# MPEGGroup/mpeg-pcc-tmc2

Hardware: AMD Instinct MI355X
Metric: encoder patch+image-gen frames/sec, longdress_vox10 32-frame GOF (higher is better)
Workload: dtype int32/f64

## Files before the change

mpeg-pcc-tmc2_amd/csrc/kdtree_device.hip:

```cpp
#include <algorithm>
#include <cstring>

#include "internal.h"

namespace tmc2 {
namespace {

constexpr uint32_t kNone      = 0xFFFFFFFFu;
constexpr int      kBlock     = 256;
constexpr int      kWaves     = kBlock / 64;
constexpr int      kScanTile  = kBlock * 8;
constexpr int      kLeafMax   = 10;
constexpr int      kMaxLevels = 64;

struct BuildSeg {
  uint32_t begin, end;
  uint32_t node, parent;
  int32_t  mn[3], mx[3];
  int16_t  lo[3], hi[3];
  uint8_t  side, pdim;
  uint8_t  split, cutDim;
  int32_t  cut;
  uint32_t mid;
  uint32_t slot;
// ... 199 lines not shown
#pragma unroll
          for ( int j = 0; j < 4; ++j ) {
            const uint32_t i = base + j * blockDim.x + threadIdx.x;
            if ( i < count ) {
              const int o = i < idx ? 0 : 6;
              if ( o == 0 ) {
                r[0] = min( r[0], int32_t( p[j].x ) ), r[1] = min( r[1], int32_t( p[j].y ) ), r[2] = min( r[2], int32_t( p[j].z ) );
                r[3] = max( r[3], int32_t( p[j].x ) ), r[4] = max( r[4], int32_t( p[j].y ) ), r[5] = max( r[5], int32_t( p[j].z ) );
              } else {
                r[6] = min( r[6], int32_t( p[j].x ) ), r[7] = min( r[7], int32_t( p[j].y ) ), r[8] = min( r[8], int32_t( p[j].z ) );
                r[9] = max( r[9], int32_t( p[j].x ) ), r[10] = max( r[10], int32_t( p[j].y ) ), r[11] = max( r[11], int32_t( p[j].z ) );
              }
            }
          }
        }
#pragma unroll
        for ( int off = 32; off > 0; off >>= 1 )
#pragma unroll
          for ( int k = 0; k < 12; ++k ) {
            const int32_t o = __shfl_xor( r[k], off, 64 );
            r[k]            = ( k % 6 ) < 3 ? min( r[k], o ) : max( r[k], o );
          }
        if ( lane == 0 )
          for ( int k = 0; k < 12; ++k ) red[wave][k] = r[k];
        __syncthreads();
        if ( threadIdx.x == 0 ) {
          for ( int w = 0; w < kHugeWaves; ++w )
            for ( int k = 0; k < 12; ++k ) r[k] = ( k % 6 ) < 3 ? min( r[k], red[w][k] ) : max( r[k], red[w][k] );
          const uint32_t id0 = atomicAdd( a.nodeCount, 2u );
          KdNode         nd;
          nd.a = int32_t( id0 ), nd.b = int32_t( id0 + 1 ), nd.divlow = int16_t( r[3 + rule.dim] ), nd.divhigh = int16_t( r[6 + rule.dim] ),
          nd.dim = rule.dim;
          a.nodes[q.node] = nd;
          HugeNode child[2];
          child[0].begin = q.begin, child[0].end = q.begin + idx, child[0].node = id0;
          child[1].begin = q.begin + idx, child[1].end = q.end, child[1].node = id0 + 1;
          for ( int c = 0; c < 2; ++c ) {
            child[c].depth = uint16_t( q.depth + 1 );
            for ( int d = 0; d < 3; ++d )
              child[c].lo[d] = lo[d], child[c].hi[d] = hi[d], child[c].mn[d] = int16_t( r[6 * c + d] ), child[c].mx[d] = int16_t( r[6 * c + 3 + d] );
          }
          const int16_t cut = int16_t( rule.cut );
          if ( rule.dim == 0 ) child[0].hi[0] = cut, child[1].lo[0] = cut;
          if ( rule.dim == 1 ) child[0].hi[1] = cut, child[1].lo[1] = cut;
          if ( rule.dim == 2 ) child[0].hi[2] = cut, child[1].lo[2] = cut;
          for ( int c = 0; c < 2; ++c ) {
            const uint32_t cc = child[c].end - child[c].begin, level = seg.level + child[c].depth;
            if ( cc <= uint32_t( kLeafMax ) ) {
              KdNode leaf;
              leaf.a = int32_t( seg.begin + child[c].begin ), leaf.b = int32_t( seg.begin + child[c].end ), leaf.divlow = leaf.divhigh = 0,
              leaf.dim = -1;
              a.nodes[child[c].node] = leaf;
              atomicMax( a.finishDepth, level + 1u );
            } else if ( cc <= a.retireMax ) {
              RetiredSeg rs;
              rs.begin = seg.begin + child[c].begin, rs.end = seg.begin + child[c].end, rs.node = child[c].node, rs.level = level, rs.root = 0;
              for ( int d = 0; d < 3; ++d ) rs.lo[d] = child[c].lo[d], rs.hi[d] = child[c].hi[d];
              a.retired[atomicAdd( a.retiredCount, 1u )] = rs;
            } else {
              sNode[cur ^ 1][sCount[cur ^ 1]++] = child[c];
            }
          }
        }
        __syncthreads();
      }
      if ( threadIdx.x == 0 ) sCount[cur] = 0;
      cur ^= 1;
      __syncthreads();
    }
  }
}

constexpr int      kPieceMax  = 4096;
constexpr int      kPieceRecs = kPieceMax / ( kLeafMax + 1 ) + 2;
constexpr uint16_t kNoRec     = 0xFFFFu;
constexpr uint32_t kNoKey     = 0xFFFFFFFFu;

struct alignas( 8 ) PieceRec {
  uint16_t begin, end;
  int16_t  cut;
  uint8_t  dim, unused0;
  uint16_t edge1, rb1;
  uint16_t edge2, rb2;
  uint16_t mid;
  uint16_t child[2];
  uint16_t unused1;
  uint32_t node;
  int32_t  lmax, rmin;
  int16_t  lo[3], hi[3];
  int32_t  mn[3], mx[3];
};
static_assert( sizeof( PieceRec ) == 72, "PieceRec layout" );
struct PieceHot0 {
  uint32_t be, dc;
};
struct PieceHot1 {
  uint32_t e1rb1, e2rb2;
};
struct PieceHot2 {
  uint32_t midc0, c1;
};

__device__ __forceinline__ void pieceBarrier() { asm volatile( "s_waitcnt lgkmcnt(0)\n\ts_barrier" ::: "memory" ); }

typedef short pkShort2 __attribute__( ( ext_vector_type( 2 ) ) );
__device__ __forceinline__ uint32_t pkMin( uint32_t a, uint32_t b ) {
  return __builtin_bit_cast( uint32_t, __builtin_elementwise_min( __builtin_bit_cast( pkShort2, a ), __builtin_bit_cast( pkShort2, b ) ) );
}
__device__ __forceinline__ uint32_t pkMax( uint32_t a, uint32_t b ) {
  return __builtin_bit_cast( uint32_t, __builtin_elementwise_max( __builtin_bit_cast( pkShort2, a ), __builtin_bit_cast( pkShort2, b ) ) );
}
__device__ __forceinline__ uint32_t pk2( int lo16, int hi16 ) { return ( uint32_t( lo16 ) & 0xFFFFu ) | ( uint32_t( hi16 ) << 16 ); }
__device__ __forceinline__ int      pkLo( uint32_t v ) { return int( int16_t( v & 0xFFFFu ) ); }
__device__ __forceinline__ int      pkHi( uint32_t v ) { return int( int16_t( v >> 16 ) ); }

template <int WAVES>
__device__ __forceinline__ uint32_t pieceScan( uint32_t v, uint32_t* waveTot ) {
  const int lane = threadIdx.x & 63, wave = threadIdx.x >> 6;
  uint32_t  inc  = v;
#pragma unroll
  for ( int off = 1; off < 64; off <<= 1 ) {
    const uint32_t t = __shfl_up( inc, off, 64 );
    if ( lane >= off ) inc += t;
  }
  if ( lane == 63 ) waveTot[wave] = inc;
  pieceBarrier();
  uint32_t before = 0;
#pragma unroll
  for ( int w = 0; w < WAVES; w += 4 ) {
    const uint4 t = *reinterpret_cast<const uint4*>( waveTot + w );
    before += ( w + 0 < wave ? t.x : 0u ) + ( w + 1 < wave ? t.y : 0u ) + ( w + 2 < wave ? t.z : 0u ) + ( w + 3 < wave ? t.w : 0u );
  }
  return before + inc - v;
}

__device__ __forceinline__ bool waveSegMinMaxPacked( uint32_t key, uint32_t& A, uint32_t& B, uint32_t& C, int lane ) {
#pragma unroll
  for ( int off = 1; off < 64; off <<= 1 ) {
    const uint32_t ok = __shfl_down( key, off, 64 );
    const uint32_t oa = __shfl_down( A, off, 64 ), ob = __shfl_down( B, off, 64 ), oc = __shfl_down( C, off, 64 );
    if ( lane + off < 64 && ok == key ) A = pkMin( A, oa ), B = pkMax( B, ob ), C = pkMin( C, oc );
  }
  const uint32_t pk = __shfl_up( key, 1, 64 );
  return key != kNoKey && ( lane == 0 || pk != key );
}

__device__ __forceinline__ void ldsMin( int32_t* slot, int32_t v ) {
  if ( v < *reinterpret_cast<volatile int32_t*>( slot ) ) atomicMin( slot, v );
}
__device__ __forceinline__ void ldsMax( int32_t* slot, int32_t v ) {
  if ( v > *reinterpret_cast<volatile int32_t*>( slot ) ) atomicMax( slot, v );
}


struct LvSeg {
  uint32_t begin, end;
  uint32_t cutInfo;
  uint32_t edge1;
  uint32_t slot;
  uint32_t childNode;
  uint32_t node, parent;
  int16_t  lo[3], hi[3];
  uint8_t  side, pdim;
  uint16_t unused;
  int32_t  mn[3], mx[3];
};

constexpr int kLandBlock = 256;
constexpr int kLandRounds = 2;
struct LvPartial {
  uint32_t slot;
  uint32_t v[6];
  uint32_t unused;
};

__device__ __forceinline__ void lvReport( LvSeg* child, int mnx, int mny, int mnz, int mxx, int mxy, int mxz ) {
  if ( mnx < loadStaleOk( &child->mn[0] ) ) atomicMin( &child->mn[0], mnx );
  if ( mny < loadStaleOk( &child->mn[1] ) ) atomicMin( &child->mn[1], mny );
  if ( mnz < loadStaleOk( &child->mn[2] ) ) atomicMin( &child->mn[2], mnz );
  if ( mxx > loadStaleOk( &child->mx[0] ) ) atomicMax( &child->mx[0], mxx );
  if ( mxy > loadStaleOk( &child->mx[1] ) ) atomicMax( &child->mx[1], mxy );
  if ( mxz > loadStaleOk( &child->mx[2] ) ) atomicMax( &child->mx[2], mxz );
}

__device__ __forceinline__ uint32_t lvPrefix( const uint32_t* __restrict__ loc, const uint32_t* sums, uint32_t tiles, uint32_t i, uint32_t n ) {
  return i < n ? loc[i] + sums[i / kScanTile] : sums[tiles];
}

__device__ __forceinline__ uint32_t lvPartner( const uint16_t* __restrict__ list, const uint32_t* sums, uint32_t from, uint32_t to, uint32_t G ) {
  uint32_t lo = from / kScanTile, hi = ( to - 1u ) / kScanTile;
  while ( lo < hi ) {
    const uint32_t mid = ( lo + hi + 1u ) / 2u;
    if ( mid * kScanTile - sums[mid] <= G )
      lo = mid;
    else
      hi = mid - 1u;
  }
  return lo * kScanTile + list[size_t( lo ) * kScanTile + ( G - ( lo * kScanTile - sums[lo] ) )];
}

__global__ __launch_bounds__( kBlock ) void lvInitKernel( BuildArgs a ) {
  __shared__ int blockRange[6 * kWaves];
  const uint32_t n = a.n, gsize = gridDim.x * blockDim.x;
  const int      lane = threadIdx.x & 63, wave = threadIdx.x >> 6;
  int mnx = 0x7FFFFFFF, mny = mnx, mnz = mnx, mxx = int( 0x80000000 ), mxy = mxx, mxz = mxx;
  for ( uint32_t i = blockIdx.x * blockDim.x + threadIdx.x; i < n; i += gsize ) {
    const Pt p = a.pts[i];
    a.P[i]     = p;
    a.perm[i]  = i;
    a.seg[i]   = 0;
    mnx = min( mnx, int( p.x ) ), mny = min( mny, int( p.y ) ), mnz = min( mnz, int( p.z ) );
    mxx = max( mxx, int( p.x ) ), mxy = max( mxy, int( p.y ) ), mxz = max( mxz, int( p.z ) );
  }
#pragma unroll
  for ( int off = 32; off > 0; off >>= 1 ) {
    mnx = min( mnx, __shfl_xor( mnx, off, 64 ) ), mny = min( mny, __shfl_xor( mny, off, 64 ) ), mnz = min( mnz, __shfl_xor( mnz, off, 64 ) );
    mxx = max( mxx, __shfl_xor( mxx, off, 64 ) ), mxy = max( mxy, __shfl_xor( mxy, off, 64 ) ), mxz = max( mxz, __shfl_xor( mxz, off, 64 ) );
  }
  if ( lane == 0 ) {
    int* w = blockRange + 6 * wave;
    w[0] = mnx, w[1] = mny, w[2] = mnz, w[3] = mxx, w[4] = mxy, w[5] = mxz;
  }
  __syncthreads();
  if ( threadIdx.x < 6 ) {
    int v = blockRange[threadIdx.x];
    for ( int w = 1; w < kWaves; ++w ) v = threadIdx.x < 3 ? min( v, blockRange[6 * w + threadIdx.x] ) : max( v, blockRange[6 * w + threadIdx.x] );
    int32_t* slot = threadIdx.x < 3 ? &a.lvA[0].mn[threadIdx.x] : &a.lvA[0].mx[threadIdx.x - 3];
    if ( threadIdx.x < 3 ) {
      if ( v < loadStaleOk( slot ) ) atomicMin( slot, v );
    } else {
      if ( v > loadStaleOk( slot ) ) atomicMax( slot, v );
    }
  }
}
__global__ void lvRootKernel( BuildArgs a ) {
  if ( threadIdx.x < kMaxLevels + 16 ) a.counts[threadIdx.x] = 0;
  __syncthreads();
  if ( threadIdx.x != 0 ) return;
  LvSeg r{};
  r.begin = 0, r.end = a.n, r.node = 0, r.parent = kNone;
  for ( int d = 0; d < 3; ++d ) r.mn[d] = 0x7FFFFFFF, r.mx[d] = int32_t( 0x80000000 );
  a.lvA[0]     = r;
  a.counts[0]  = 1;
  *a.nodeCount = 1;
}

constexpr int kDecideThreads = 1024;
constexpr int kDecideRng     = 2000;
__global__ __launch_bounds__( kDecideThreads ) void lvDecideKernel( BuildArgs a, uint32_t level ) {
  __shared__ uint32_t waveTot[kDecideThreads / 64];
  __shared__ uint32_t sCarry;
  __shared__ int32_t  sRng[kDecideRng][6];
  LvSeg*         cur   = ( level & 1 ) ? a.lvB : a.lvA;
  const uint32_t count = a.counts[level], nodeBase = *a.nodeCount;
  const int      lane = threadIdx.x & 63, wave = threadIdx.x >> 6;
  if ( threadIdx.x == 0 ) sCarry = 0;
  const bool inLds = level > 0 && count <= a.decideRng;
  if ( inLds ) {
    for ( uint32_t t = threadIdx.x; t < count * 6u; t += kDecideThreads ) sRng[t / 6u][t % 6u] = ( t % 6u ) < 3u ? 0x7FFFFFFF : int32_t( 0x80000000 );
    __syncthreads();
  }
  if ( level > 0 ) {
    const uint32_t nPart = ( a.n + uint32_t( kLandBlock * kLandRounds ) - 1u ) / uint32_t( kLandBlock * kLandRounds );
    for ( uint32_t base = 0; base < nPart; base += kDecideThreads ) {
      const uint32_t t = base + threadIdx.x;
      LvPartial      pt;
      pt.slot = kNone;
      if ( t < nPart ) pt = a.partial[t];
#pragma unroll
      for ( int c = 0; c < 2; ++c ) {
        uint32_t A = pt.v[3 * c], B = pt.v[3 * c + 1], C = pt.v[3 * c + 2];
        if ( waveSegMinMaxPacked( pt.slot == kNone ? kNoKey : pt.slot, A, B, C, lane ) ) {
          if ( inLds ) {
            int32_t* r = sRng[pt.slot + c];
            ldsMin( &r[0], pkLo( A ) ), ldsMin( &r[1], pkHi( A ) ), ldsMin( &r[2], pkLo( C ) );
            ldsMax( &r[3], pkLo( B ) ), ldsMax( &r[4], pkHi( B ) ), ldsMax( &r[5], ~pkHi( C ) );
          } else {
            lvReport( cur + pt.slot + c, pkLo( A ), pkHi( A ), pkLo( C ), pkLo( B ), pkHi( B ), ~pkHi( C ) );
          }
        }
      }
    }
    if ( !inLds ) asm volatile( "s_waitcnt vmcnt(0)" ::: "memory" );
  }
  __syncthreads();
  for ( uint32_t base = 0; base < count; base += kDecideThreads ) {
    const uint32_t s     = base + threadIdx.x;
    uint32_t       split = 0;
    LvSeg*         q     = cur + s;
    if ( s < count ) {
      const bool root = q->parent == kNone;
      int32_t    mn[3], mx[3], lo[3], hi[3];
#pragma unroll
      for ( int d = 0; d < 3; ++d ) {
        mn[d] = __hip_atomic_load( &q->mn[d], __ATOMIC_RELAXED, __HIP_MEMORY_SCOPE_AGENT );
        mx[d] = __hip_atomic_load( &q->mx[d], __ATOMIC_RELAXED, __HIP_MEMORY_SCOPE_AGENT );
        if ( inLds ) mn[d] = min( mn[d], sRng[s][d] ), mx[d] = max( mx[d], sRng[s][3 + d] );
        lo[d] = root ? mn[d] : int32_t( q->lo[d] );
        hi[d] = root ? mx[d] : int32_t( q->hi[d] );
      }
      if ( root ) {
        for ( int d = 0; d < 3; ++d ) a.rootBox[d] = mn[d], a.rootBox[3 + d] = mx[d];
      } else {
        const int pd = q->pdim;
        if ( q->side == 0 )
          a.nodes[q->parent].divlow = int16_t( pd == 0 ? mx[0] : ( pd == 1 ? mx[1] : mx[2] ) );
// ... 173 lines not shown
    if ( i == b ) q->edge1 = edge;
    if ( i >= edge || coordOf( pi, int( ( ci >> 16 ) & 0xFFu ) ) < int32_t( int16_t( ci & 0xFFFFu ) ) ) continue;
    const uint32_t r  = li + lvSums[i / kScanTile] - rb;
    const uint32_t j  = lvPartner( a.list, lvSums, edge, e, ( e - re ) - 1u - r );
    const Pt       pj = a.P[j];
    a.P[i]            = pj;
    a.P[j]            = pi;
    const uint32_t u  = a.perm[i];
    a.perm[i]         = a.perm[j];
    a.perm[j]         = u;
  }
}

__global__ __launch_bounds__( kLandBlock ) void lvSwapTwoKernel( BuildArgs a, uint32_t level ) {
  extern __shared__ uint32_t lvSums[];
  const uint32_t n = a.n, tiles = a.tiles;
  const int      lane  = threadIdx.x & 63;
  LvSeg*         cur  = ( level & 1 ) ? a.lvB : a.lvA;
  LvSeg*         next = ( level & 1 ) ? a.lvA : a.lvB;
  lvLoadSums<kLandBlock>( lvSums, a.tile2, tiles );
  const uint32_t nRound = ( n + uint32_t( kLandBlock ) - 1u ) & ~( uint32_t( kLandBlock ) - 1u );
  __shared__ uint32_t blockSeg;
  __shared__ uint32_t red[kLandBlock / 64][6];
  __shared__ uint32_t accV[6], accSlot;
  const int wave = threadIdx.x >> 6;
  constexpr uint32_t kChunk = uint32_t( kLandBlock ) * kLandRounds;
  for ( uint32_t c0 = blockIdx.x * kChunk; c0 < nRound; c0 += gridDim.x * kChunk ) {
  if ( threadIdx.x == 0 ) accSlot = kNone;
  for ( uint32_t i0 = c0; i0 < min( c0 + kChunk, nRound ); i0 += kLandBlock ) {
    const uint32_t i   = i0 + threadIdx.x;
    uint32_t       key = kNoKey;
    uint32_t       A = pk2( 0x7FFF, 0x7FFF ), B = pk2( -0x8000, -0x8000 ), C = pk2( 0x7FFF, 0x7FFF );
    uint32_t       A2 = A, B2 = B, C2 = C;
    bool           moved = false;
    uint32_t       s = kNone, slot = 0;
    if ( i < n ) {
      s           = a.seg[i];
      uint32_t to = kNone;
      if ( s != kNone ) {
        LvSeg*         q  = cur + s;
        const uint32_t ci = q->cutInfo;
        if ( ci >> 24 ) {
          const uint32_t b = q->begin, e = q->end, e1 = q->edge1;
          slot               = q->slot;
          const int      dim = int( ( ci >> 16 ) & 0xFFu );
          const int32_t  cut = int32_t( int16_t( ci & 0xFFFFu ) );
          Pt             pi  = a.P[i];
          const uint32_t li  = a.loc2[i];
          const uint32_t rb = lvPrefix( a.loc2, lvSums, tiles, e1, n ), re = lvPrefix( a.loc2, lvSums, tiles, e, n );
          const uint32_t e2   = e1 + ( ( e - e1 ) - ( re - rb ) );
          const uint32_t cnt  = e - b, half = cnt / 2, lim1 = e1 - b, lim2 = e2 - b;
          const uint32_t idx  = lim1 > half ? lim1 : ( lim2 < half ? lim2 : half );
          const uint32_t mid  = b + idx;
          if ( i == b ) {
            KdNode nd;
            nd.a = int32_t( q->childNode ), nd.b = int32_t( q->childNode + 1u ), nd.divlow = nd.divhigh = 0, nd.dim = dim;
            a.nodes[q->node] = nd;
            for ( int c = 0; c < 2; ++c ) {
              LvSeg* ch = next + slot + c;
              ch->begin = c ? mid : b, ch->end = c ? e : mid, ch->cutInfo = 0, ch->edge1 = 0, ch->slot = 0, ch->childNode = 0;
              ch->node = q->childNode + c, ch->parent = q->node, ch->side = uint8_t( c ), ch->pdim = uint8_t( dim ), ch->unused = 0;
              for ( int d = 0; d < 3; ++d ) ch->lo[d] = q->lo[d], ch->hi[d] = q->hi[d];
              if ( c == 0 ) {
                if ( dim == 0 ) ch->hi[0] = int16_t( cut );
                if ( dim == 1 ) ch->hi[1] = int16_t( cut );
                if ( dim == 2 ) ch->hi[2] = int16_t( cut );
              } else {
                if ( dim == 0 ) ch->lo[0] = int16_t( cut );
                if ( dim == 1 ) ch->lo[1] = int16_t( cut );
                if ( dim == 2 ) ch->lo[2] = int16_t( cut );
              }
            }
          }
          const int32_t x = coordOf( pi, dim );
          to              = slot + ( i >= mid ? 1u : 0u );
          key             = to;
          if ( i >= e1 && i < e2 && x > cut ) {
            const uint32_t r  = li + lvSums[i / kScanTile] - rb;
            const uint32_t j  = lvPartner( a.list, lvSums, e2, e, ( e - re ) - 1u - r );
            const Pt       pj = a.P[j];
            a.P[i]            = pj;
            a.P[j]            = pi;
            const uint32_t u  = a.perm[i];
            a.perm[i]         = a.perm[j];
            a.perm[j]         = u;
            moved             = true;
            A2 = pk2( pi.x, pi.y ), B2 = A2, C2 = pk2( pi.z, ~int( pi.z ) );
            pi = pj;
          }
          if ( !( i >= e2 && x <= cut ) ) A = pk2( pi.x, pi.y ), B = A, C = pk2( pi.z, ~int( pi.z ) );
        }
        a.seg[i] = to;
      }
    }
    if ( threadIdx.x == 0 ) blockSeg = s;
    __syncthreads();
    const bool uniform = __syncthreads_and( s == blockSeg ) != 0;
    if ( uniform ) {
      const bool anything = __syncthreads_or( key != kNoKey ) != 0;
      if ( anything ) {
        uint32_t v[6];
        const bool right = key != kNoKey && key != slot;
        v[0] = right || key == kNoKey ? pk2( 0x7FFF, 0x7FFF ) : A, v[1] = right || key == kNoKey ? pk2( -0x8000, -0x8000 ) : B,
        v[2] = right || key == kNoKey ? pk2( 0x7FFF, 0x7FFF ) : C;
        v[3] = pkMin( right ? A : pk2( 0x7FFF, 0x7FFF ), A2 ), v[4] = pkMax( right ? B : pk2( -0x8000, -0x8000 ), B2 ),
        v[5] = pkMin( right ? C : pk2( 0x7FFF, 0x7FFF ), C2 );
#pragma unroll
        for ( int off = 32; off > 0; off >>= 1 ) {
          v[0] = pkMin( v[0], __shfl_xor( v[0], off, 64 ) ), v[1] = pkMax( v[1], __shfl_xor( v[1], off, 64 ) ), v[2] = pkMin( v[2], __shfl_xor( v[2], off, 64 ) );
          v[3] = pkMin( v[3], __shfl_xor( v[3], off, 64 ) ), v[4] = pkMax( v[4], __shfl_xor( v[4], off, 64 ) ), v[5] = pkMin( v[5], __shfl_xor( v[5], off, 64 ) );
        }
        if ( lane == 0 )
          for ( int k = 0; k < 6; ++k ) red[wave][k] = v[k];
        __syncthreads();
        if ( threadIdx.x == 0 ) {
          uint32_t x[6];
          for ( int k = 0; k < 6; ++k ) {
            x[k] = red[0][k];
            for ( int w = 1; w < kLandBlock / 64; ++w ) x[k] = ( k % 3 ) == 1 ? pkMax( x[k], red[w][k] ) : pkMin( x[k], red[w][k] );
          }
          if ( accSlot != kNone && accSlot != slot ) {
            for ( int c = 0; c < 2; ++c )
              lvReport( next + accSlot + c, pkLo( accV[3 * c] ), pkHi( accV[3 * c] ), pkLo( accV[3 * c + 2] ), pkLo( accV[3 * c + 1] ), pkHi( accV[3 * c + 1] ),
                        ~pkHi( accV[3 * c + 2] ) );
            accSlot = kNone;
          }
          for ( int k = 0; k < 6; ++k ) accV[k] = accSlot == kNone ? x[k] : ( ( k % 3 ) == 1 ? pkMax( accV[k], x[k] ) : pkMin( accV[k], x[k] ) );
          accSlot = slot;
        }
      }
      __syncthreads();
      continue;
    }
    if ( moved ) lvReport( next + slot + 1u, pkLo( A2 ), pkHi( A2 ), pkLo( C2 ), pkLo( A2 ), pkHi( A2 ), pkLo( C2 ) );
    if ( waveSegMinMaxPacked( key, A, B, C, lane ) )
      lvReport( next + key, pkLo( A ), pkHi( A ), pkLo( C ), pkLo( B ), pkHi( B ), ~pkHi( C ) );
  }
  __syncthreads();
  if ( threadIdx.x == 0 ) {
    LvPartial pt;
    pt.slot = accSlot, pt.unused = 0;
    for ( int k = 0; k < 6; ++k ) pt.v[k] = accV[k];
    a.partial[c0 / kChunk] = pt;
  }
  __syncthreads();
  }
}

constexpr size_t kPieceLdsBytes = size_t( kPieceMax ) * ( sizeof( Pt ) + 4 + 2 + 2 + 2 ) + 16 + 2 * size_t( kPieceRecs ) * sizeof( PieceRec );

constexpr int kPiecePer = 4;
template <bool PROFILE = false>
__global__ __launch_bounds__( kPieceMax / kPiecePer ) void pieceKernel( BuildArgs a ) {
  unsigned long long profLast = 0, prof[12] = {0, 0, 0, 0, 0, 0, 0, 0, 0, 0, 0, 0};
#define PIECE_MARK( k )                                        \
  if ( PROFILE && threadIdx.x == 0 ) {                         \
    const unsigned long long now_ = wall_clock64();            \
    prof[k] += now_ - profLast, profLast = now_;               \
  }
  constexpr int K = kPiecePer, THREADS = kPieceMax / K, WAVES = THREADS / 64;
  extern __shared__ __align__( 16 ) unsigned char pieceLds[];
  Pt*       P     = reinterpret_cast<Pt*>( pieceLds );
  uint32_t* perm  = reinterpret_cast<uint32_t*>( P + kPieceMax );
  uint16_t* pre   = reinterpret_cast<uint16_t*>( perm + kPieceMax );
  uint16_t* lst   = pre + kPieceMax + 8;
  uint16_t* segOf = lst + kPieceMax;
  PieceRec* recs  = reinterpret_cast<PieceRec*>( segOf + kPieceMax );
  __shared__ __align__( 16 ) uint32_t sWave[2][WAVES];
  __shared__ uint32_t sCount[2], sNodeBase, sDepth;
  const int      lane = threadIdx.x & 63, tid = threadIdx.x;
  const uint32_t total = *a.retiredCount;
  const uint32_t p0    = uint32_t( tid ) * K;
  for ( uint32_t s = blockIdx.x; s < total; s += gridDim.x ) {
    const RetiredSeg seg = a.retired[s];
    const uint32_t   cnt = seg.end - seg.begin;
    uint32_t idPending   = 0;
    if ( tid == 0 ) idPending = atomicAdd( a.nodeCount, 2u );
    pieceBarrier();
    for ( uint32_t i = tid; i < uint32_t( kPieceMax ); i += THREADS ) {
      if ( i < cnt ) {
        P[i]     = a.P[seg.begin + i];
        perm[i]  = a.perm[seg.begin + i];
        segOf[i] = 0;
      } else {
        segOf[i] = kNoRec;
      }
    }
    if ( tid == 0 ) {
      PieceRec r{};
      r.begin = 0, r.end = uint16_t( cnt ), r.node = seg.node;
      for ( int d = 0; d < 3; ++d ) r.lo[d] = seg.lo[d], r.hi[d] = seg.hi[d], r.mn[d] = 0x7FFFFFFF, r.mx[d] = int32_t( 0x80000000 );
      recs[0]   = r;
      sCount[0] = 1, sCount[1] = 0, sDepth = 0;
    }
    pieceBarrier();
    {
      uint32_t A = pk2( 0x7FFF, 0x7FFF ), B = pk2( -0x8000, -0x8000 ), C = pk2( 0x7FFF, 0x7FFF );
      bool     any = false;
#pragma unroll
      for ( int k = 0; k < K; ++k ) {
        const uint32_t p = p0 + k;
        if ( p < cnt ) {
          const Pt x = P[p];
          A = pkMin( A, pk2( x.x, x.y ) ), B = pkMax( B, pk2( x.x, x.y ) ), C = pkMin( C, pk2( x.z, ~int( x.z ) ) );
          any = true;
        }
      }
      if ( waveSegMinMaxPacked( any ? 0u : kNoKey, A, B, C, lane ) ) {
        ldsMin( &recs[0].mn[0], pkLo( A ) ), ldsMin( &recs[0].mn[1], pkHi( A ) ), ldsMin( &recs[0].mn[2], pkLo( C ) );
        ldsMax( &recs[0].mx[0], pkLo( B ) ), ldsMax( &recs[0].mx[1], pkHi( B ) ), ldsMax( &recs[0].mx[2], ~pkHi( C ) );
      }
    }
    pieceBarrier();
    if ( seg.root != 0 && tid == 0 ) {
      for ( int d = 0; d < 3; ++d ) {
        recs[0].lo[d] = int16_t( recs[0].mn[d] ), recs[0].hi[d] = int16_t( recs[0].mx[d] );
        a.rootBox[d] = recs[0].mn[d], a.rootBox[3 + d] = recs[0].mx[d];
      }
    }
    if ( PROFILE && threadIdx.x == 0 ) profLast = wall_clock64();
    uint32_t deepest  = 0;
    uint32_t prevBase = 0, prevCount = 0;
    int      cur      = 0;
    for ( uint32_t depth = 0;; ++depth ) {
      pieceBarrier();
      PIECE_MARK( 0 )
      const uint32_t nc = sCount[cur];
      PieceRec*      R  = recs + cur * kPieceRecs;
      PieceRec*      RN = recs + ( cur ^ 1 ) * kPieceRecs;
      for ( uint32_t r = tid; r < prevCount; r += THREADS ) {
        const PieceRec* q = RN + r;
        KdNode          nd;
        nd.a = int32_t( prevBase + 2u * r ), nd.b = int32_t( prevBase + 2u * r + 1u ), nd.divlow = int16_t( q->lmax ), nd.divhigh = int16_t( q->rmin ),
        nd.dim = q->dim;
        a.nodes[q->node] = nd;
      }
      if ( nc == 0 ) break;
      if ( seg.level + depth >= uint32_t( kMaxLevels ) - 2u ) {
        if ( tid == 0 ) atomicMax( a.finishDepth, 0x10000u );
        break;
      }
      if ( tid == 0 ) sNodeBase = idPending, sCount[cur ^ 1] = 0;
      for ( uint32_t r = tid; r < nc; r += THREADS ) {
        PieceRec*     q   = R + r;
        const int32_t lo0 = q->lo[0], lo1 = q->lo[1], lo2 = q->lo[2], hi0 = q->hi[0], hi1 = q->hi[1], hi2 = q->hi[2];
        const int32_t mn0 = q->mn[0], mn1 = q->mn[1], mn2 = q->mn[2], mx0 = q->mx[0], mx1 = q->mx[1], mx2 = q->mx[2];
        const int32_t maxSpan = max( hi0 - lo0, max( hi1 - lo1, hi2 - lo2 ) );
        const double  limit   = ( 1.0 - 0.00001 ) * double( maxSpan );
        int           dim     = 0;
        int32_t       best    = -1;
        if ( double( hi0 - lo0 ) > limit && mx0 - mn0 > best ) best = mx0 - mn0, dim = 0;
        if ( double( hi1 - lo1 ) > limit && mx1 - mn1 > best ) best = mx1 - mn1, dim = 1;
        if ( double( hi2 - lo2 ) > limit && mx2 - mn2 > best ) best = mx2 - mn2, dim = 2;
        const int32_t l = dim == 0 ? lo0 : ( dim == 1 ? lo1 : lo2 ), h = dim == 0 ? hi0 : ( dim == 1 ? hi1 : hi2 );
        const int32_t lowest = dim == 0 ? mn0 : ( dim == 1 ? mn1 : mn2 ), highest = dim == 0 ? mx0 : ( dim == 1 ? mx1 : mx2 );
        q->dim = uint8_t( dim ), q->unused0 = 0, q->cut = int16_t( min( max( ( l + h ) / 2, lowest ), highest ) );
      }
      pieceBarrier();
      PIECE_MARK( 1 )
      uint32_t rec[K], be[K], dc[K];
      bool     waveLive = true;
      {
        uint16_t raw[K];
        *reinterpret_cast<uint2*>( raw ) = *reinterpret_cast<const uint2*>( segOf + p0 );
        bool same = true, live = false;
#pragma unroll
        for ( int k = 0; k < K; ++k ) rec[k] = raw[k], same = same && raw[k] == raw[0], live = live || raw[k] != kNoRec;
        waveLive = __ballot( live ) != 0ull;
        if ( same ) {
          PieceHot0 h{0, 0};
          if ( rec[0] != kNoRec ) h = *reinterpret_cast<const PieceHot0*>( R + rec[0] );
#pragma unroll
          for ( int k = 0; k < K; ++k ) be[k] = h.be, dc[k] = h.dc;
        } else {
#pragma unroll
          for ( int k = 0; k < K; ++k ) {
            PieceHot0 h{0, 0};
            if ( rec[k] != kNoRec ) h = *reinterpret_cast<const PieceHot0*>( R + rec[k] );
            be[k] = h.be, dc[k] = h.dc;
          }
        }
      }
      uint32_t f1 = 0;
      if ( waveLive ) {
        Pt x[K];
#pragma unroll
        for ( int k = 0; k < K; k += 2 ) *reinterpret_cast<uint4*>( &x[k] ) = *reinterpret_cast<const uint4*>( P + p0 + k );
#pragma unroll
        for ( int k = 0; k < K; ++k ) {
          const int d = int( ( dc[k] >> 16 ) & 0xFFu ), c = int( int16_t( dc[k] & 0xFFFFu ) );
          const int v = int( int16_t( __builtin_bit_cast( uint64_t, x[k] ) >> ( 16 * d ) ) );
          if ( rec[k] != kNoRec && v >= c ) f1 |= 1u << k;
        }
      }
      uint32_t preA[K + 1];
      {
        uint32_t at = pieceScan<WAVES>( uint32_t( __popc( f1 ) ), sWave[0] );
        uint16_t out[K];
#pragma unroll
        for ( int k = 0; k < K; ++k ) preA[k] = at, out[k] = uint16_t( at ), at += ( f1 >> k ) & 1u;
        preA[K] = at;
        *reinterpret_cast<uint2*>( pre + p0 ) = *reinterpret_cast<const uint2*>( out );
        if ( tid == THREADS - 1 ) pre[kPieceMax] = uint16_t( at );
      }
      pieceBarrier();
      PIECE_MARK( 2)
      uint32_t edge1[K], rb1[K];
#pragma unroll
      for ( int k = 0; k < K; ++k ) {
        edge1[k] = rb1[k] = 0;
        if ( !waveLive || rec[k] == kNoRec ) continue;
        if ( k > 0 && rec[k] == rec[k - 1] ) {
          edge1[k] = edge1[k - 1], rb1[k] = rb1[k - 1];
        } else {
          const uint32_t b = be[k] & 0xFFFFu, e = be[k] >> 16, rb = pre[b], re = pre[e];
          edge1[k] = b + ( ( e - b ) - ( re - rb ) ), rb1[k] = rb | ( re << 16 );
        }
        const uint32_t p = p0 + k, b = be[k] & 0xFFFFu, e = be[k] >> 16;
        if ( p >= edge1[k] && !( ( f1 >> k ) & 1u ) ) lst[b + ( ( e - p - 1u ) - ( ( rb1[k] >> 16 ) - preA[k + 1] ) )] = uint16_t( p );
        if ( p == b ) *reinterpret_cast<uint32_t*>( &R[rec[k]].edge1 ) = edge1[k] | ( ( rb1[k] & 0xFFFFu ) << 16 );
      }
      pieceBarrier();
      PIECE_MARK( 3)
#pragma unroll
      for ( int k = 0; k < K; ++k ) {
        const uint32_t p = p0 + k;
        if ( waveLive && rec[k] != kNoRec && p < edge1[k] && ( ( f1 >> k ) & 1u ) ) {
          const uint32_t j  = lst[( be[k] & 0xFFFFu ) + ( preA[k] - ( rb1[k] & 0xFFFFu ) )];
          const Pt       px = P[p], pj = P[j];
          const uint32_t ip = perm[p], ij = perm[j];
          P[p] = pj, P[j] = px, perm[p] = ij, perm[j] = ip;
        }
      }
      pieceBarrier();
      PIECE_MARK( 4)
      uint32_t f2 = 0;
      if ( waveLive ) {
        Pt x[K];
#pragma unroll
        for ( int k = 0; k < K; k += 2 ) *reinterpret_cast<uint4*>( &x[k] ) = *reinterpret_cast<const uint4*>( P + p0 + k );
#pragma unroll
        for ( int k = 0; k < K; ++k ) {
          const int d = int( ( dc[k] >> 16 ) & 0xFFu ), c = int( int16_t( dc[k] & 0xFFFFu ) );
          const int v = int( int16_t( __builtin_bit_cast( uint64_t, x[k] ) >> ( 16 * d ) ) );
          if ( rec[k] != kNoRec && p0 + k >= edge1[k] && v > c ) f2 |= 1u << k;
        }
      }
      {
        uint32_t at = pieceScan<WAVES>( uint32_t( __popc( f2 ) ), sWave[1] );
        uint16_t out[K];
#pragma unroll
        for ( int k = 0; k < K; ++k ) preA[k] = at, out[k] = uint16_t( at ), at += ( f2 >> k ) & 1u;
        preA[K] = at;
        *reinterpret_cast<uint2*>( pre + p0 ) = *reinterpret_cast<const uint2*>( out );
        if ( tid == THREADS - 1 ) pre[kPieceMax] = uint16_t( at );
      }
      pieceBarrier();
      PIECE_MARK( 5)
      const uint32_t base = sNodeBase;
      for ( uint32_t r = tid; r < nc; r += THREADS ) {
        PieceRec*      q  = R + r;
        const uint32_t b = q->begin, e = q->end, e1 = q->edge1, rb2 = pre[e1], re2 = pre[e];
        const uint32_t e2   = e1 + ( ( e - e1 ) - ( re2 - rb2 ) );
        const uint32_t n    = e - b, half = n / 2, lim1 = e1 - b, lim2 = e2 - b;
        const uint32_t idx  = lim1 > half ? lim1 : ( lim2 < half ? lim2 : half );
        const uint32_t mid  = b + idx;
        const uint32_t id0  = base + 2u * r;
        const int      dim  = q->dim;
        const int16_t  cut  = q->cut;
        q->edge2 = uint16_t( e2 ), q->rb2 = uint16_t( rb2 ), q->mid = uint16_t( mid );
        q->lmax = int32_t( 0x80000000 ), q->rmin = 0x7FFFFFFF;
#pragma unroll
        for ( int c = 0; c < 2; ++c ) {
          const uint32_t cb = c ? mid : b, ce = c ? e : mid;
          if ( ce - cb <= uint32_t( kLeafMax ) ) {
            KdNode leaf;
            leaf.a = int32_t( seg.begin + cb ), leaf.b = int32_t( seg.begin + ce ), leaf.divlow = leaf.divhigh = 0, leaf.dim = -1;
            a.nodes[id0 + c] = leaf;
            q->child[c]      = kNoRec;
            deepest          = max( deepest, seg.level + depth + 2u );
          } else {
            const uint32_t slot = atomicAdd( &sCount[cur ^ 1], 1u );
            PieceRec*      ch   = RN + slot;
            ch->begin = uint16_t( cb ), ch->end = uint16_t( ce ), ch->node = id0 + c;
            int16_t l0 = q->lo[0], l1 = q->lo[1], l2 = q->lo[2], h0 = q->hi[0], h1 = q->hi[1], h2 = q->hi[2];
            if ( c == 0 ) {
              if ( dim == 0 ) h0 = cut;
              if ( dim == 1 ) h1 = cut;
              if ( dim == 2 ) h2 = cut;
            } else {
              if ( dim == 0 ) l0 = cut;
              if ( dim == 1 ) l1 = cut;
              if ( dim == 2 ) l2 = cut;
            }
            ch->lo[0] = l0, ch->lo[1] = l1, ch->lo[2] = l2, ch->hi[0] = h0, ch->hi[1] = h1, ch->hi[2] = h2;
            ch->mn[0] = ch->mn[1] = ch->mn[2] = 0x7FFFFFFF, ch->mx[0] = ch->mx[1] = ch->mx[2] = int32_t( 0x80000000 );
            q->child[c] = uint16_t( slot );
          }
        }
      }
      uint32_t edge2[K], rb2[K];
#pragma unroll
      for ( int k = 0; k < K; ++k ) {
        edge2[k] = rb2[k] = 0;
        if ( !waveLive || rec[k] == kNoRec ) continue;
        const uint32_t e = be[k] >> 16, e1 = edge1[k];
        if ( k > 0 && rec[k] == rec[k - 1] ) {
          edge2[k] = edge2[k - 1], rb2[k] = rb2[k - 1];
        } else {
          const uint32_t rb = pre[e1], re = pre[e];
          edge2[k] = e1 + ( ( e - e1 ) - ( re - rb ) ), rb2[k] = rb | ( re << 16 );
        }
        const uint32_t p = p0 + k;
        if ( p >= edge2[k] && !( ( f2 >> k ) & 1u ) ) lst[e1 + ( ( e - p - 1u ) - ( ( rb2[k] >> 16 ) - preA[k + 1] ) )] = uint16_t( p );
      }
      pieceBarrier();
      PIECE_MARK( 6)
      prevBase = base, prevCount = nc;
      if ( tid == 0 && sCount[cur ^ 1] ) idPending = atomicAdd( a.nodeCount, 2u * sCount[cur ^ 1] );
#pragma unroll
      for ( int k = 0; k < K; ++k ) {
        const uint32_t p = p0 + k;
        if ( waveLive && rec[k] != kNoRec && p >= edge1[k] && p < edge2[k] && ( ( f2 >> k ) & 1u ) ) {
          const uint32_t j  = lst[edge1[k] + ( preA[k] - ( rb2[k] & 0xFFFFu ) )];
          const Pt       px = P[p], pj = P[j];
          const uint32_t ip = perm[p], ij = perm[j];
          P[p] = pj, P[j] = px, perm[p] = ij, perm[j] = ip;
        }
      }
      pieceBarrier();
      PIECE_MARK( 7)
      if ( waveLive ) {
        uint32_t key[K], mc[K], c1[K];
        bool     same = true;
#pragma unroll
        for ( int k = 0; k < K; ++k ) {
          mc[k] = c1[k] = 0;
          if ( rec[k] != kNoRec ) {
            if ( k > 0 && rec[k] == rec[k - 1] ) {
              mc[k] = mc[k - 1], c1[k] = c1[k - 1];
            } else {
              const PieceHot2 h = *reinterpret_cast<const PieceHot2*>( &R[rec[k]].mid );
              mc[k] = h.midc0, c1[k] = h.c1 & 0xFFFFu;
            }
          }
          key[k] = rec[k] == kNoRec ? kNoKey : 2u * rec[k] + ( p0 + k >= ( mc[k] & 0xFFFFu ) ? 1u : 0u );
          same   = same && key[k] == key[0];
        }
        Pt x[K];
#pragma unroll
        for ( int k = 0; k < K; k += 2 ) *reinterpret_cast<uint4*>( &x[k] ) = *reinterpret_cast<const uint4*>( P + p0 + k );
        uint32_t A = pk2( 0x7FFF, 0x7FFF ), B = pk2( -0x8000, -0x8000 ), C = pk2( 0x7FFF, 0x7FFF );
        if ( same && key[0] != kNoKey ) {
#pragma unroll
          for ( int k = 0; k < K; ++k )
            A = pkMin( A, pk2( x[k].x, x[k].y ) ), B = pkMax( B, pk2( x[k].x, x[k].y ) ), C = pkMin( C, pk2( x[k].z, ~int( x[k].z ) ) );
        }
        const bool head = waveSegMinMaxPacked( same ? key[0] : kNoKey, A, B, C, lane );
        uint16_t out[K];
#pragma unroll
        for ( int k = 0; k < K; ++k ) {
          out[k] = kNoRec;
          if ( key[k] == kNoKey ) continue;
          const uint32_t side = key[k] & 1u;
          const uint32_t cr   = side ? c1[k] : ( mc[k] >> 16 );
          out[k]              = uint16_t( cr );
          if ( same ? ( k > 0 || !head ) : false ) continue;
          int mnx, mny, mnz, mxx, mxy, mxz;
          if ( same )
            mnx = pkLo( A ), mny = pkHi( A ), mnz = pkLo( C ), mxx = pkLo( B ), mxy = pkHi( B ), mxz = ~pkHi( C );
          else
            mnx = mxx = x[k].x, mny = mxy = x[k].y, mnz = mxz = x[k].z;
          PieceRec* q = R + rec[k];
          const int d = int( ( dc[k] >> 16 ) & 0xFFu );
          if ( side == 0 )
            ldsMax( &q->lmax, d == 0 ? mxx : ( d == 1 ? mxy : mxz ) );
          else
            ldsMin( &q->rmin, d == 0 ? mnx : ( d == 1 ? mny : mnz ) );
          if ( cr != kNoRec ) {
            PieceRec* ch = RN + cr;
            ldsMin( &ch->mn[0], mnx ), ldsMin( &ch->mn[1], mny ), ldsMin( &ch->mn[2], mnz );
            ldsMax( &ch->mx[0], mxx ), ldsMax( &ch->mx[1], mxy ), ldsMax( &ch->mx[2], mxz );
          }
        }
        *reinterpret_cast<uint2*>( segOf + p0 ) = *reinterpret_cast<const uint2*>( out );
      }
      cur ^= 1;
    }
    if ( deepest ) atomicMax( &sDepth, deepest );
    if ( PROFILE && threadIdx.x == 0 ) {
      for ( int k = 0; k < 8; ++k ) atomicAdd( a.pieceProfile + k, prof[k] ), prof[k] = 0;
      atomicAdd( a.pieceProfile + 8, 1ull );
    }
    pieceBarrier();
    for ( uint32_t i = tid; i < cnt; i += THREADS ) {
      a.P[seg.begin + i]    = P[i];
      a.perm[seg.begin + i] = perm[i];
    }
    if ( tid == 0 && sDepth ) atomicMax( a.finishDepth, sDepth );
  }
  if ( a.hostDepth && tid == 0 ) {
    __threadfence();
    if ( atomicAdd( a.ticket, 1u ) == gridDim.x - 1u ) {
      __threadfence();
      *a.hostDepth = __hip_atomic_load( a.finishDepth, __ATOMIC_RELAXED, __HIP_MEMORY_SCOPE_AGENT );
    }
  }
}

}

int buildKdTreeDevice( tmc2_ctx* ctx, const Pt* d_pts, uint64_t n64, DeviceTree& tree ) {
  const uint32_t n = uint32_t( n64 );
  tree.n           = n64;
  tree.depth       = 0;
  for ( int d = 0; d < 3; ++d ) tree.lo[d] = tree.hi[d] = 0;
  if ( n == 0 ) return TMC2_OK;
  hipStream_t    s       = ctx->stream;
  const uint32_t tiles   = ( n + kScanTile - 1 ) / kScanTile;
  const size_t   maxSegs = 2 * ( size_t( n ) / ( kLeafMax + 1 ) + 1 ) + 2;
  const size_t   maxNode = 2 * size_t( n ) + 2;
  TMC2_TRY( tree.ptsTree.alloc( n ) );
  TMC2_TRY( tree.perm.alloc( n ) );
  TMC2_TRY( tree.nodes.alloc( maxNode ) );
  DevBuf<uint32_t>   d_work, d_small;
  DevBuf<BuildSeg>   d_segs;
  DevBuf<RetiredSeg> d_retired;
  const size_t       maxRetired = size_t( n ) / ( kLeafMax + 1 ) + 2;
  TMC2_TRY( d_retired.alloc( maxRetired ) );
  DevBuf<HugeSeg> d_huge;
  TMC2_TRY( d_huge.alloc( size_t( n ) / ( kPieceMax + 1 ) + 2 ) );
  const auto     hugeEnv = ctxOption( ctx, "KD_HUGEMAX" );
  const uint32_t hugeMax = std::min<uint32_t>( kHugeLimit, std::max<uint32_t>( kPieceMax, hugeEnv ? uint32_t( atoi( hugeEnv->c_str() ) ) : 16384u ) );
  TMC2_TRY( d_work.alloc( 3 * size_t( n ) + 2 * ( size_t( tiles ) + 1 ) ) );
  TMC2_TRY( d_segs.alloc( 2 * maxSegs ) );
  TMC2_TRY( d_small.alloc( kMaxLevels + 16 ) );
  static_assert( kMaxLevels + 16 <= 128, "lvRootKernel clears the counters with one workgroup of 128" );
  BuildArgs a;
  a.pts = d_pts, a.n = n, a.tiles = tiles, a.P = tree.ptsTree.p, a.perm = tree.perm.p;
  a.seg = d_work.p, a.loc1 = d_work.p + n, a.loc2 = d_work.p + 2 * size_t( n );
  a.tile1 = d_work.p + 3 * size_t( n ), a.tile2 = a.tile1 + tiles + 1;
  a.segA = d_segs.p, a.segB = d_segs.p + maxSegs, a.nodes = tree.nodes.p;
  a.counts    = d_small.p;
  a.nodeCount = d_small.p + kMaxLevels + 1;
  a.levels    = d_small.p + kMaxLevels + 2;
  a.rootBox   = reinterpret_cast<int32_t*>( d_small.p + kMaxLevels + 8 );
  a.retired      = d_retired.p;
  a.retiredCount = d_small.p + kMaxLevels + 3;
  a.finishDepth  = d_small.p + kMaxLevels + 4;
  a.ticket       = d_small.p + kMaxLevels + 5;
  a.bigCount     = d_small.p + kMaxLevels + 6;
  a.huge         = d_huge.p;
  a.hugeCount    = d_small.p + kMaxLevels + 7;
  a.hugeMax      = hugeMax;
  a.hostSmall    = nullptr;
  a.hostDepth    = ctx->answerLine( tmc2_ctx::kAnswerTreeDepth );
  a.retireMax    = uint32_t( kPieceMax );
  a.splitMax     = uint32_t( kPieceMax );
  const dim3 blk( kBlock ), grdE( std::max<uint32_t>( 1u, ( n + 2 * kBlock - 1 ) / ( 2 * kBlock ) ) ), grdT( tiles );
  const dim3 grdL( std::max<uint32_t>( 1u, ( n + kLandBlock * kLandRounds - 1 ) / ( kLandBlock * kLandRounds ) ) );
  const size_t sumsLds = ( size_t( tiles ) + 1 ) * 4;
  if ( sumsLds > 48 * 1024 ) {
    setError( "kdtree: %u points -- the level passes hold one word per 2 048-point tile in LDS (at most 25 M points)", n );
    return TMC2_E_UNSUPPORTED;
  }
  DevBuf<LvSeg>    d_lv;
  DevBuf<uint16_t> d_list;
  DevBuf<LvPartial> d_partial;
  const size_t     maxLv = 2 * ( size_t( n ) / ( size_t( kPieceMax ) + 1 ) + 2 );
  TMC2_TRY( d_lv.alloc( 2 * maxLv ) );
  TMC2_TRY( d_list.alloc( size_t( tiles ) * kScanTile ) );
  TMC2_TRY( d_partial.alloc( size_t( n ) / ( kLandBlock * kLandRounds ) + 2 ) );
  a.lvA = d_lv.p, a.lvB = d_lv.p + maxLv, a.list = d_list.p, a.partial = d_partial.p;
  const auto decideOpt = ctxOption( ctx, "KD_DECIDE" );
  a.decideRng = decideOpt && ( *decideOpt )[0] == 'g' ? 0u : uint32_t( kDecideRng );
  hipLaunchKernelGGL( lvRootKernel, dim3( 1 ), dim3( 128 ), 0, s, a );
  hipLaunchKernelGGL( lvInitKernel, dim3( std::min<uint32_t>( grdE.x, 1024u ) ), blk, 0, s, a );
  hipLaunchKernelGGL( lvDecideKernel, dim3( 1 ), dim3( kDecideThreads ), 0, s, a, 0u );
  uint32_t out[kMaxLevels + 16];
  int      found = -1;
  int& hint = ctx->kdLevelHint[( n >> 15 ) * 2u + 1u];
  for ( uint32_t level = 0; level < uint32_t( kMaxLevels ) && found < 0; ) {
    uint32_t chunkEnd = level + 1;
    if ( level == 0 && hint > 0 ) {
      chunkEnd = uint32_t( std::min( hint, kMaxLevels ) );
    } else {
      while ( chunkEnd < uint32_t( kMaxLevels ) && ( uint64_t( hugeMax ) << std::min<uint32_t>( chunkEnd - 1, 40 ) ) < n ) ++chunkEnd;
      if ( chunkEnd == level + 1 ) chunkEnd = std::min<uint32_t>( level + 2, kMaxLevels );
    }
    volatile uint32_t* hostSmall = ctx->answerLine( tmc2_ctx::kAnswerTreeLevels );
    for ( ; level < chunkEnd; ++level ) {
      hipLaunchKernelGGL( lvFlagKernel<true>, grdT, blk, 0, s, a, level );
      hipLaunchKernelGGL( lvSwapOneKernel, grdE, blk, sumsLds, s, a, level );
      hipLaunchKernelGGL( lvFlagKernel<false>, grdT, blk, 0, s, a, level );
      hipLaunchKernelGGL( lvSwapTwoKernel, grdL, dim3( kLandBlock ), sumsLds, s, a, level );
      BuildArgs ad = a;
      if ( level + 1 == chunkEnd ) ad.hostSmall = hostSmall;
      hipLaunchKernelGGL( lvDecideKernel, dim3( 1 ), dim3( kDecideThreads ), 0, s, ad, level + 1u );
    }
    TMC2_HIP( hipGetLastError() );
    TMC2_HIP( hipStreamSynchronize( s ) );
    for ( int w = 0; w < kMaxLevels + 16; ++w ) out[w] = hostSmall[w];
    for ( uint32_t l = 0; l <= level && l <= uint32_t( kMaxLevels ); ++l )
      if ( out[l] == 0 ) {
        found = int( l );
        break;
      }
  }
  if ( found < 0 ) {
    setError( "kdtree: more than %d levels", kMaxLevels - 1 );
    return TMC2_E_UNSUPPORTED;
  }
  tree.depth = found;
  hint       = std::max( found, 1 );
  const int32_t* box = reinterpret_cast<const int32_t*>( out + kMaxLevels + 8 );
  for ( int d = 0; d < 3; ++d ) tree.lo[d] = box[d], tree.hi[d] = box[3 + d];
  const uint32_t hugeSegs = out[kMaxLevels + 7];
  if ( hugeSegs )
    hipLaunchKernelGGL( hugeSegmentsKernel, dim3( std::min<uint32_t>( hugeSegs, 4u * uint32_t( ctx->cuCount ) ) ), dim3( 64 * kHugeWaves ), 0, s, a );
  const uint32_t retired = out[kMaxLevels + 3] + hugeSegs * ( 2u * hugeMax / uint32_t( kPieceMax ) );
  if ( retired ) {
    const dim3 grid( std::min<uint32_t>( retired, 8u * uint32_t( ctx->cuCount ) ) ), block( kPieceMax / kPiecePer );
    if ( ctxOption( ctx, "KD_PIECE_PROFILE" ) ) {
      DevBuf<unsigned long long> d_prof;
      TMC2_TRY( d_prof.alloc( 16 ) );
      TMC2_HIP( hipMemsetAsync( d_prof.p, 0, 16 * 8, s ) );
      a.pieceProfile = d_prof.p;
      TMC2_TRY( allowLargeLds( reinterpret_cast<const void*>( pieceKernel<true> ), kPieceLdsBytes, ctx->device, 256 ) );
      hipLaunchKernelGGL( pieceKernel<true>, grid, block, kPieceLdsBytes, s, a );
      unsigned long long h[16];
      TMC2_HIP( hipMemcpyAsync( h, d_prof.p, sizeof( h ), hipMemcpyDeviceToHost, s ) );
      TMC2_HIP( hipStreamSynchronize( s ) );
      static const char* what[8] = {"landing of the previous depth", "node records + split rules", "first flags + prefix sum", "first publish",
                                    "first swaps", "second flags + prefix sum", "children + second publish", "second swaps"};
      fprintf( stderr, "pieceKernel: %llu pieces, us per piece between the barriers of its depths (thread 0 of each workgroup):", h[8] );
      for ( int k = 0; k < 8; ++k ) fprintf( stderr, " %s %.1f |", what[k], 0.01 * double( h[k] ) / double( std::max<unsigned long long>( h[8], 1 ) ) );
      fprintf( stderr, "\n" );
    } else {
      TMC2_TRY( allowLargeLds( reinterpret_cast<const void*>( pieceKernel<> ), kPieceLdsBytes, ctx->device, 256 ) );
      hipLaunchKernelGGL( pieceKernel<>, grid, block, kPieceLdsBytes, s, a );
    }
    TMC2_HIP( hipGetLastError() );
    TMC2_HIP( hipStreamSynchronize( s ) );
    const uint32_t fin = *a.hostDepth;
    if ( fin >= uint32_t( kMaxLevels ) ) {
      setError( "kdtree: more than %d levels", kMaxLevels - 1 );
      return TMC2_E_UNSUPPORTED;
    }
    tree.depth = std::max( tree.depth, int( fin ) );
  }
  return TMC2_OK;
}

}
```

Before: 194.7.

## Keep piece points in registers and fuse second swap into landing phase

The kd-tree piece kernel now keeps each thread's points in registers across depths and reloads them from LDS only when a swap partner may have changed them. The second swap pass is merged into the landing phase, which removes one workgroup barrier per depth. Swapped-out points feed their bounds straight into the child records with atomics. The conditional-read guard in front of the LDS min/max atomics is dropped in favour of plain atomics. This cuts LDS reloads and barriers, but adds more complex staleness tracking and more unconditional atomics.

```diff
diff --git a/mpeg-pcc-tmc2_amd/csrc/kdtree_device.hip b/mpeg-pcc-tmc2_amd/csrc/kdtree_device.hip
--- a/mpeg-pcc-tmc2_amd/csrc/kdtree_device.hip
+++ b/mpeg-pcc-tmc2_amd/csrc/kdtree_device.hip
@@ -375,6 +375,11 @@
   if ( v > *reinterpret_cast<volatile int32_t*>( slot ) ) atomicMax( slot, v );
 }
 
+__device__ __forceinline__ void pieceMin( int32_t* slot, int32_t v ) { atomicMin( slot, v ); }
+__device__ __forceinline__ void pieceMax( int32_t* slot, int32_t v ) { atomicMax( slot, v ); }
+__device__ __forceinline__ uint32_t ptXY( uint64_t q ) { return uint32_t( q ); }
+__device__ __forceinline__ uint32_t ptZnZ( uint64_t q ) { return ( uint32_t( q >> 32 ) & 0xFFFFu ) | ( ~uint32_t( q >> 32 ) << 16 ); }
+__device__ __forceinline__ int      ptCoord( uint64_t q, int d ) { return int( int16_t( q >> ( 16 * d ) ) ); }
 
 struct LvSeg {
   uint32_t begin, end;
@@ -854,7 +859,7 @@
 constexpr int kPiecePer = 4;
 template <bool PROFILE = false>
 __global__ __launch_bounds__( kPieceMax / kPiecePer ) void pieceKernel( BuildArgs a ) {
-  unsigned long long profLast = 0, prof[12] = {0, 0, 0, 0, 0, 0, 0, 0, 0, 0, 0, 0};
+  unsigned long long profLast = 0, prof[8] = {0, 0, 0, 0, 0, 0, 0, 0};
 #define PIECE_MARK( k )                                        \
   if ( PROFILE && threadIdx.x == 0 ) {                         \
     const unsigned long long now_ = wall_clock64();            \
@@ -863,6 +868,7 @@
   constexpr int K = kPiecePer, THREADS = kPieceMax / K, WAVES = THREADS / 64;
   extern __shared__ __align__( 16 ) unsigned char pieceLds[];
   Pt*       P     = reinterpret_cast<Pt*>( pieceLds );
+  uint64_t* P64   = reinterpret_cast<uint64_t*>( pieceLds );
   uint32_t* perm  = reinterpret_cast<uint32_t*>( P + kPieceMax );
   uint16_t* pre   = reinterpret_cast<uint16_t*>( perm + kPieceMax );
   uint16_t* lst   = pre + kPieceMax + 8;
@@ -896,6 +902,10 @@
       sCount[0] = 1, sCount[1] = 0, sDepth = 0;
     }
     pieceBarrier();
+    uint64_t x[K];
+    uint32_t stale = 0;
+#pragma unroll
+    for ( int k = 0; k < K; k += 2 ) *reinterpret_cast<uint4*>( &x[k] ) = *reinterpret_cast<const uint4*>( P + p0 + k );
     {
       uint32_t A = pk2( 0x7FFF, 0x7FFF ), B = pk2( -0x8000, -0x8000 ), C = pk2( 0x7FFF, 0x7FFF );
       bool     any = false;
@@ -903,14 +913,13 @@
       for ( int k = 0; k < K; ++k ) {
         const uint32_t p = p0 + k;
         if ( p < cnt ) {
-          const Pt x = P[p];
-          A = pkMin( A, pk2( x.x, x.y ) ), B = pkMax( B, pk2( x.x, x.y ) ), C = pkMin( C, pk2( x.z, ~int( x.z ) ) );
+          A = pkMin( A, ptXY( x[k] ) ), B = pkMax( B, ptXY( x[k] ) ), C = pkMin( C, ptZnZ( x[k] ) );
           any = true;
         }
       }
       if ( waveSegMinMaxPacked( any ? 0u : kNoKey, A, B, C, lane ) ) {
-        ldsMin( &recs[0].mn[0], pkLo( A ) ), ldsMin( &recs[0].mn[1], pkHi( A ) ), ldsMin( &recs[0].mn[2], pkLo( C ) );
-        ldsMax( &recs[0].mx[0], pkLo( B ) ), ldsMax( &recs[0].mx[1], pkHi( B ) ), ldsMax( &recs[0].mx[2], ~pkHi( C ) );
+        pieceMin( &recs[0].mn[0], pkLo( A ) ), pieceMin( &recs[0].mn[1], pkHi( A ) ), pieceMin( &recs[0].mn[2], pkLo( C ) );
+        pieceMax( &recs[0].mx[0], pkLo( B ) ), pieceMax( &recs[0].mx[1], pkHi( B ) ), pieceMax( &recs[0].mx[2], ~pkHi( C ) );
       }
     }
     pieceBarrier();
@@ -985,13 +994,15 @@
       }
       uint32_t f1 = 0;
       if ( waveLive ) {
-        Pt x[K];
-#pragma unroll
-        for ( int k = 0; k < K; k += 2 ) *reinterpret_cast<uint4*>( &x[k] ) = *reinterpret_cast<const uint4*>( P + p0 + k );
+        if ( stale ) {
+#pragma unroll
+          for ( int k = 0; k < K; k += 2 ) *reinterpret_cast<uint4*>( &x[k] ) = *reinterpret_cast<const uint4*>( P + p0 + k );
+          stale = 0;
+        }
 #pragma unroll
         for ( int k = 0; k < K; ++k ) {
           const int d = int( ( dc[k] >> 16 ) & 0xFFu ), c = int( int16_t( dc[k] & 0xFFFFu ) );
-          const int v = int( int16_t( __builtin_bit_cast( uint64_t, x[k] ) >> ( 16 * d ) ) );
+          const int v = ptCoord( x[k], d );
           if ( rec[k] != kNoRec && v >= c ) f1 |= 1u << k;
         }
       }
@@ -1027,24 +1038,30 @@
 #pragma unroll
       for ( int k = 0; k < K; ++k ) {
         const uint32_t p = p0 + k;
-        if ( waveLive && rec[k] != kNoRec && p < edge1[k] && ( ( f1 >> k ) & 1u ) ) {
+        if ( !waveLive || rec[k] == kNoRec ) continue;
+        if ( p < edge1[k] && ( ( f1 >> k ) & 1u ) ) {
           const uint32_t j  = lst[( be[k] & 0xFFFFu ) + ( preA[k] - ( rb1[k] & 0xFFFFu ) )];
-          const Pt       px = P[p], pj = P[j];
+          const uint64_t pj = P64[j];
           const uint32_t ip = perm[p], ij = perm[j];
-          P[p] = pj, P[j] = px, perm[p] = ij, perm[j] = ip;
+          P64[p] = pj, P64[j] = x[k], perm[p] = ij, perm[j] = ip;
+          x[k] = pj;
+        } else if ( p >= edge1[k] && !( ( f1 >> k ) & 1u ) ) {
+          stale |= 1u << k;
         }
       }
       pieceBarrier();
       PIECE_MARK( 4)
       uint32_t f2 = 0;
       if ( waveLive ) {
-        Pt x[K];
-#pragma unroll
-        for ( int k = 0; k < K; k += 2 ) *reinterpret_cast<uint4*>( &x[k] ) = *reinterpret_cast<const uint4*>( P + p0 + k );
+        if ( stale ) {
+#pragma unroll
+          for ( int k = 0; k < K; k += 2 ) *reinterpret_cast<uint4*>( &x[k] ) = *reinterpret_cast<const uint4*>( P + p0 + k );
+          stale = 0;
+        }
 #pragma unroll
         for ( int k = 0; k < K; ++k ) {
           const int d = int( ( dc[k] >> 16 ) & 0xFFu ), c = int( int16_t( dc[k] & 0xFFFFu ) );
-          const int v = int( int16_t( __builtin_bit_cast( uint64_t, x[k] ) >> ( 16 * d ) ) );
+          const int v = ptCoord( x[k], d );
           if ( rec[k] != kNoRec && p0 + k >= edge1[k] && v > c ) f2 |= 1u << k;
         }
       }
@@ -1120,20 +1137,8 @@
       PIECE_MARK( 6)
       prevBase = base, prevCount = nc;
       if ( tid == 0 && sCount[cur ^ 1] ) idPending = atomicAdd( a.nodeCount, 2u * sCount[cur ^ 1] );
-#pragma unroll
-      for ( int k = 0; k < K; ++k ) {
-        const uint32_t p = p0 + k;
-        if ( waveLive && rec[k] != kNoRec && p >= edge1[k] && p < edge2[k] && ( ( f2 >> k ) & 1u ) ) {
-          const uint32_t j  = lst[edge1[k] + ( preA[k] - ( rb2[k] & 0xFFFFu ) )];
-          const Pt       px = P[p], pj = P[j];
-          const uint32_t ip = perm[p], ij = perm[j];
-          P[p] = pj, P[j] = px, perm[p] = ij, perm[j] = ip;
-        }
-      }
-      pieceBarrier();
-      PIECE_MARK( 7)
       if ( waveLive ) {
-        uint32_t key[K], mc[K], c1[K];
+        uint32_t key[K], mc[K], c1[K], gone = 0;
         bool     same = true;
 #pragma unroll
         for ( int k = 0; k < K; ++k ) {
@@ -1149,14 +1154,36 @@
           key[k] = rec[k] == kNoRec ? kNoKey : 2u * rec[k] + ( p0 + k >= ( mc[k] & 0xFFFFu ) ? 1u : 0u );
           same   = same && key[k] == key[0];
         }
-        Pt x[K];
-#pragma unroll
-        for ( int k = 0; k < K; k += 2 ) *reinterpret_cast<uint4*>( &x[k] ) = *reinterpret_cast<const uint4*>( P + p0 + k );
+#pragma unroll
+        for ( int k = 0; k < K; ++k ) {
+          const uint32_t p = p0 + k;
+          if ( rec[k] == kNoRec || p < edge1[k] ) continue;
+          if ( p < edge2[k] && ( ( f2 >> k ) & 1u ) ) {
+            const uint32_t j  = lst[edge1[k] + ( preA[k] - ( rb2[k] & 0xFFFFu ) )];
+            const uint64_t px = x[k], pj = P64[j];
+            const uint32_t ip = perm[p], ij = perm[j];
+            P64[p] = pj, P64[j] = px, perm[p] = ij, perm[j] = ip;
+            x[k] = pj;
+            PieceRec* q = R + rec[k];
+            const int d = int( ( dc[k] >> 16 ) & 0xFFu );
+            pieceMin( &q->rmin, ptCoord( px, d ) );
+            if ( c1[k] != kNoRec ) {
+              PieceRec* ch = RN + c1[k];
+              const int vx = ptCoord( px, 0 ), vy = ptCoord( px, 1 ), vz = ptCoord( px, 2 );
+              pieceMin( &ch->mn[0], vx ), pieceMin( &ch->mn[1], vy ), pieceMin( &ch->mn[2], vz );
+              pieceMax( &ch->mx[0], vx ), pieceMax( &ch->mx[1], vy ), pieceMax( &ch->mx[2], vz );
+            }
+          } else if ( p >= edge2[k] && !( ( f2 >> k ) & 1u ) ) {
+            gone |= 1u << k;
+          }
+        }
+        stale = gone;
         uint32_t A = pk2( 0x7FFF, 0x7FFF ), B = pk2( -0x8000, -0x8000 ), C = pk2( 0x7FFF, 0x7FFF );
         if ( same && key[0] != kNoKey ) {
 #pragma unroll
           for ( int k = 0; k < K; ++k )
-            A = pkMin( A, pk2( x[k].x, x[k].y ) ), B = pkMax( B, pk2( x[k].x, x[k].y ) ), C = pkMin( C, pk2( x[k].z, ~int( x[k].z ) ) );
+            if ( !( ( gone >> k ) & 1u ) )
+              A = pkMin( A, ptXY( x[k] ) ), B = pkMax( B, ptXY( x[k] ) ), C = pkMin( C, ptZnZ( x[k] ) );
         }
         const bool head = waveSegMinMaxPacked( same ? key[0] : kNoKey, A, B, C, lane );
         uint16_t out[K];
@@ -1167,22 +1194,22 @@
           const uint32_t side = key[k] & 1u;
           const uint32_t cr   = side ? c1[k] : ( mc[k] >> 16 );
           out[k]              = uint16_t( cr );
-          if ( same ? ( k > 0 || !head ) : false ) continue;
+          if ( same ? ( k > 0 || !head ) : bool( ( gone >> k ) & 1u ) ) continue;
           int mnx, mny, mnz, mxx, mxy, mxz;
           if ( same )
             mnx = pkLo( A ), mny = pkHi( A ), mnz = pkLo( C ), mxx = pkLo( B ), mxy = pkHi( B ), mxz = ~pkHi( C );
           else
-            mnx = mxx = x[k].x, mny = mxy = x[k].y, mnz = mxz = x[k].z;
+            mnx = mxx = ptCoord( x[k], 0 ), mny = mxy = ptCoord( x[k], 1 ), mnz = mxz = ptCoord( x[k], 2 );
           PieceRec* q = R + rec[k];
           const int d = int( ( dc[k] >> 16 ) & 0xFFu );
           if ( side == 0 )
-            ldsMax( &q->lmax, d == 0 ? mxx : ( d == 1 ? mxy : mxz ) );
+            pieceMax( &q->lmax, d == 0 ? mxx : ( d == 1 ? mxy : mxz ) );
           else
-            ldsMin( &q->rmin, d == 0 ? mnx : ( d == 1 ? mny : mnz ) );
+            pieceMin( &q->rmin, d == 0 ? mnx : ( d == 1 ? mny : mnz ) );
           if ( cr != kNoRec ) {
             PieceRec* ch = RN + cr;
-            ldsMin( &ch->mn[0], mnx ), ldsMin( &ch->mn[1], mny ), ldsMin( &ch->mn[2], mnz );
-            ldsMax( &ch->mx[0], mxx ), ldsMax( &ch->mx[1], mxy ), ldsMax( &ch->mx[2], mxz );
+            pieceMin( &ch->mn[0], mnx ), pieceMin( &ch->mn[1], mny ), pieceMin( &ch->mn[2], mnz );
+            pieceMax( &ch->mx[0], mxx ), pieceMax( &ch->mx[1], mxy ), pieceMax( &ch->mx[2], mxz );
           }
         }
         *reinterpret_cast<uint2*>( segOf + p0 ) = *reinterpret_cast<const uint2*>( out );
@@ -1333,10 +1360,10 @@
       unsigned long long h[16];
       TMC2_HIP( hipMemcpyAsync( h, d_prof.p, sizeof( h ), hipMemcpyDeviceToHost, s ) );
       TMC2_HIP( hipStreamSynchronize( s ) );
-      static const char* what[8] = {"landing of the previous depth", "node records + split rules", "first flags + prefix sum", "first publish",
-                                    "first swaps", "second flags + prefix sum", "children + second publish", "second swaps"};
+      static const char* what[7] = {"second swaps + landing of the previous depth", "node records + split rules", "first flags + prefix sum", "first publish",
+                                    "first swaps", "second flags + prefix sum", "children + second publish"};
       fprintf( stderr, "pieceKernel: %llu pieces, us per piece between the barriers of its depths (thread 0 of each workgroup):", h[8] );
-      for ( int k = 0; k < 8; ++k ) fprintf( stderr, " %s %.1f |", what[k], 0.01 * double( h[k] ) / double( std::max<unsigned long long>( h[8], 1 ) ) );
+      for ( int k = 0; k < 7; ++k ) fprintf( stderr, " %s %.1f |", what[k], 0.01 * double( h[k] ) / double( std::max<unsigned long long>( h[8], 1 ) ) );
       fprintf( stderr, "\n" );
     } else {
       TMC2_TRY( allowLargeLds( reinterpret_cast<const void*>( pieceKernel<> ), kPieceLdsBytes, ctx->device, 256 ) );
```

After: 195.3 (median of 3 runs). No clear change (+0.3%).
